# d9d-project/d9d

Measured on AMD Instinct MI355X. Metric: tokens/sec (whole node), Qwen3-MoE pretrain, higher is better.
Workload: dtype bf16; 1 GPU; model=qwen3-moe-16L-768h-128e-top8 (reference example/qwen3_moe/pretrain.json), global_batch=128, seq_len=4096, microbatch=8, parallelism=dp1, optimizer=StochasticAdamW bf16+SR, engine=raw

## Files before the change

d9d_amd/csrc/attention.hip:

```cpp
#include "common.h"
#include "mfma.h"

#include <torch/extension.h>
#include <ATen/hip/HIPContext.h>

#include <type_traits>

namespace d9d {

constexpr int kFwdQ = 128;
constexpr int kFwdKv = 64;
constexpr int kBwdQ = 64;
constexpr int kBwdKv = 128;
constexpr int kBwdThreads = 512;
constexpr float kLog2e = 1.44269504088896340736f;

template <int D>
constexpr int swz_rm_mask() {
  constexpr int mask = D == 128 ? 15 : (D == 64 ? 7 : 3);
  static_assert((D * 2) % (16 * (mask + 1)) == 0, "swizzle leaves its LDS row");
  return mask;
}

template <int D, typename Byte>
D9D_DEVICE Byte* swz_rm_at(Byte* tile, int row, int col) {
  return tile + row * (D * 2) + ((col * 2) ^ ((row & swz_rm_mask<D>()) << 4));
}

template <int ROWS, typename Byte>
D9D_DEVICE Byte* swz_t_at(Byte* tile, int d, int r) {
  static_assert((ROWS * 2) % (16 << 3) == 0, "swizzle leaves its LDS row");
  return tile + d * (ROWS * 2) + ((r * 2) ^ ((d & 7) << 4));
}

template <int D, int BLOCK = 256>
D9D_DEVICE void transpose_lds_tile(bf16_t* dst, const bf16_t* src_rm, int tid) {
  for (int idx = tid; idx < (64 / 4) * (D / 2); idx += BLOCK) {
    const int d0 = (idx / 16) * 2;
    const int rb = (idx % 16) * 4;
    bf16x4_bits c0, c1;
#pragma unroll
    for (int i = 0; i < 4; ++i) {
      const uint32_t pair = *reinterpret_cast<const uint32_t*>(
          swz_rm_at<D>(reinterpret_cast<const char*>(src_rm), rb + i, d0));
      c0.s[i] = (ushort)(pair & 0xffffu);
      c1.s[i] = (ushort)(pair >> 16);
    }
    *reinterpret_cast<uint64_t*>(
        swz_t_at<64>(reinterpret_cast<char*>(dst), d0, rb)) = c0.u;
    *reinterpret_cast<uint64_t*>(
        swz_t_at<64>(reinterpret_cast<char*>(dst), d0 + 1, rb)) = c1.u;
  }
}

template <int D>
D9D_DEVICE void load_transposed_block(
    bf16x4_bits& c0, bf16x4_bits& c1, const bf16_t* src, int64_t row_stride,
    int row_lo, int row0, int row_clamp, int idx) {
  const int d0 = (idx % (D / 2)) * 2;
  const int rb = (idx / (D / 2)) * 4;
#pragma unroll
  for (int i = 0; i < 4; ++i) {
    const int g_row = row_lo + min(row0 + rb + i, row_clamp);
    const uint32_t pair = *reinterpret_cast<const uint32_t*>(
        src + (int64_t)g_row * row_stride + d0);
    c0.s[i] = (ushort)(pair & 0xffffu);
    c1.s[i] = (ushort)(pair >> 16);
  }
}

template <int D, int ROWS>
D9D_DEVICE void store_transposed_block(
    bf16_t* dst, const bf16x4_bits& c0, const bf16x4_bits& c1, int idx) {
  const int d0 = (idx % (D / 2)) * 2;
  const int rb = (idx / (D / 2)) * 4;
  *reinterpret_cast<uint64_t*>(
      swz_t_at<ROWS>(reinterpret_cast<char*>(dst), d0, rb)) = c0.u;
  *reinterpret_cast<uint64_t*>(
      swz_t_at<ROWS>(reinterpret_cast<char*>(dst), d0 + 1, rb)) = c1.u;
}

template <int D, int ROWS, int BLOCK>
D9D_DEVICE void stage_transposed_tile(
    bf16_t* dst, const bf16_t* src, int64_t row_stride,
    int row_lo, int row0, int row_clamp, int tid) {
  for (int idx = tid; idx < (ROWS / 4) * (D / 2); idx += BLOCK) {
    bf16x4_bits c0, c1;
    load_transposed_block<D>(c0, c1, src, row_stride, row_lo, row0, row_clamp, idx);
    store_transposed_block<D, ROWS>(dst, c0, c1, idx);
  }
}


struct TileLoc {
  int b, h, tile;
  int q_lo, Sq_loc, kv_lo, Skv_loc;
  int causal_off;
  bool valid;
};

template <int TILE, bool TILE_KV>
D9D_DEVICE TileLoc locate_tile(
    const int* __restrict__ cu_q, const int* __restrict__ cu_k,
    const int* __restrict__ tile_pref, int nseq,
    int Sq, int Skv, int Hq, int q_offset) {
  TileLoc t;
  if (cu_q != nullptr) {
    t.h = blockIdx.y;
    int lo = 0, hi = nseq - 1;
    while (lo < hi) {
      const int mid = (lo + hi + 1) >> 1;
      if (tile_pref[mid] <= (int)blockIdx.x) lo = mid; else hi = mid - 1;
    }
    t.b = 0;
    t.tile = blockIdx.x - tile_pref[lo];
    t.q_lo = cu_q[lo];
    t.Sq_loc = cu_q[lo + 1] - t.q_lo;
    t.kv_lo = cu_k[lo];
    t.Skv_loc = cu_k[lo + 1] - t.kv_lo;
    t.causal_off = t.Skv_loc - t.Sq_loc + q_offset;
    t.valid = t.tile * TILE < (TILE_KV ? t.Skv_loc : t.Sq_loc);
  } else {
    const int wid = xcd_remap(blockIdx.y * gridDim.x + blockIdx.x,
                              gridDim.x * gridDim.y);
    const int bh = wid / gridDim.x;
    t.b = bh / Hq;
    t.h = bh % Hq;
    t.tile = wid % gridDim.x;
    t.q_lo = 0; t.Sq_loc = Sq; t.kv_lo = 0; t.Skv_loc = Skv;
    t.causal_off = q_offset;
    t.valid = true;
  }
  return t;
}

D9D_DEVICE bool causal_window_masked(bool masked, int q_pos, int kv_pos,
                                     int causal, int window_left) {
  if (causal) masked |= kv_pos > q_pos;
  if (window_left >= 0) masked |= kv_pos < q_pos - window_left;
  return masked;
}


template <int D>
__global__ __launch_bounds__(256, 2) void flash_fwd_kernel(
    const bf16_t* __restrict__ q,
    const bf16_t* __restrict__ k,
    const bf16_t* __restrict__ v,
    bf16_t* __restrict__ out,
    float* __restrict__ lse,
    const float* __restrict__ sinks,
    const int* __restrict__ cu_q,
    const int* __restrict__ cu_k,
    const int* __restrict__ qtile_pref,
    int nseq,
    int B, int Sq, int Skv, int Hq, int Hkv,
    float scale, int causal, int window_left, int q_offset) {
  constexpr int kNT = D / 16;
  constexpr int kKS = D / 32;

  extern __shared__ __attribute__((aligned(16))) char smem[];
  bf16_t* k_lds = reinterpret_cast<bf16_t*>(smem);
  bf16_t* vt_lds = k_lds + kFwdKv * D;
  bf16_t* p_lds = vt_lds + D * kFwdKv;

  const int lane = threadIdx.x & 63;
  const int wave = threadIdx.x >> 6;

  const TileLoc loc = locate_tile<kFwdQ, false>(
      cu_q, cu_k, qtile_pref, nseq, Sq, Skv, Hq, q_offset);
  if (!loc.valid) return;
  const int b = loc.b, h = loc.h, q_tile = loc.tile, causal_off = loc.causal_off;
  const int q_lo = loc.q_lo, Sq_loc = loc.Sq_loc, kv_lo = loc.kv_lo, Skv_loc = loc.Skv_loc;
  const int hkv = h / (Hq / Hkv);

  const int64_t q_base = ((int64_t)b * Sq * Hq + h) * D;
  const int64_t kv_base = ((int64_t)b * Skv * Hkv + hkv) * D;
  const int64_t q_row_stride = (int64_t)Hq * D;
  const int64_t kv_row_stride = (int64_t)Hkv * D;

  bf16x8 q_frag[2][kKS];
#pragma unroll
  for (int m = 0; m < 2; ++m) {
    const int q_row_local = q_tile * kFwdQ + wave * 32 + m * 16 + (lane & 15);
    const int safe_row = q_lo + min(q_row_local, Sq_loc - 1);
    const bf16_t* qp = q + q_base + (int64_t)safe_row * q_row_stride;
#pragma unroll
    for (int ks = 0; ks < kKS; ++ks) {
      q_frag[m][ks] = *reinterpret_cast<const bf16x8*>(qp + ks * 32 + (lane >> 4) * 8);
    }
  }

  const float m_init = sinks ? sinks[h] : -1e30f;
  const float l_init = (sinks && (threadIdx.x & 15) == 0) ? 1.f : 0.f;
  float m_run[2][4], l_run[2][4];
#pragma unroll
  for (int m = 0; m < 2; ++m)
#pragma unroll
    for (int r = 0; r < 4; ++r) {
      m_run[m][r] = m_init;
      l_run[m][r] = l_init;
    }
  f32x4 o_acc[2][kNT];
#pragma unroll
  for (int m = 0; m < 2; ++m)
#pragma unroll
    for (int nt = 0; nt < kNT; ++nt) o_acc[m][nt] = {0.f, 0.f, 0.f, 0.f};

  const int q_tile_last_row = min(q_tile * kFwdQ + kFwdQ - 1, Sq_loc - 1);
  int kv_end = Skv_loc;
  if (causal) kv_end = min(Skv_loc, q_tile_last_row + causal_off + 1);
  const int num_kv_tiles = (kv_end + kFwdKv - 1) / kFwdKv;
  if (num_kv_tiles <= 0) return;

  constexpr int kKIters = (kFwdKv * D) / (256 * 8);
  constexpr int kVIters = (kFwdKv / 4) * (D / 2) / 256;
  bf16x8 k_reg[kKIters];
  bf16x4_bits v_c0[kVIters], v_c1[kVIters];

  auto load_regs = [&](int kt) {
    const int kv0 = kt * kFwdKv;
#pragma unroll
    for (int it = 0; it < kKIters; ++it) {
      const int idx = (threadIdx.x + it * 256) * 8;
      const int row = idx / D;
      const int col = idx % D;
      const int g_row = kv_lo + min(kv0 + row, Skv_loc - 1);
      k_reg[it] = *reinterpret_cast<const bf16x8*>(
          k + kv_base + (int64_t)g_row * kv_row_stride + col);
    }
#pragma unroll
    for (int it = 0; it < kVIters; ++it) {
      load_transposed_block<D>(v_c0[it], v_c1[it], v + kv_base, kv_row_stride,
                               kv_lo, kv0, Skv_loc - 1, threadIdx.x + it * 256);
    }
  };

  auto store_lds = [&]() {
#pragma unroll
    for (int it = 0; it < kKIters; ++it) {
      const int idx = (threadIdx.x + it * 256) * 8;
      *reinterpret_cast<bf16x8*>(
          swz_rm_at<D>(reinterpret_cast<char*>(k_lds), idx / D, idx % D)) =
          k_reg[it];
    }
#pragma unroll
    for (int it = 0; it < kVIters; ++it) {
      store_transposed_block<D, kFwdKv>(vt_lds, v_c0[it], v_c1[it],
                                        threadIdx.x + it * 256);
    }
  };

  load_regs(0);
  store_lds();
  __syncthreads();

  for (int kt = 0; kt < num_kv_tiles; ++kt) {
    const int kv0 = kt * kFwdKv;
    if (kt + 1 < num_kv_tiles) load_regs(kt + 1);

#pragma unroll
    for (int m = 0; m < 2; ++m) {
      f32x4 s_acc[4];
#pragma unroll
      for (int nt = 0; nt < 4; ++nt) s_acc[nt] = {0.f, 0.f, 0.f, 0.f};
      __builtin_amdgcn_s_setprio(1);
#pragma unroll
      for (int nt = 0; nt < 4; ++nt) {
        const int kv_row = nt * 16 + (lane & 15);
#pragma unroll
        for (int ks = 0; ks < kKS; ++ks) {
          const int d0 = ks * 32 + (lane >> 4) * 8;
          const bf16x8 kb = *reinterpret_cast<const bf16x8*>(
              swz_rm_at<D>(reinterpret_cast<char*>(k_lds), kv_row, d0));
          s_acc[nt] = mfma16(q_frag[m][ks], kb, s_acc[nt]);
        }
      }
      __builtin_amdgcn_s_setprio(0);

      const int my_q_row = q_tile * kFwdQ + wave * 32 + m * 16;
      float p_val[4][4];
      float m_new[4];
#pragma unroll
      for (int r = 0; r < 4; ++r) m_new[r] = m_run[m][r];
      const int row_lo = my_q_row + causal_off;
      const bool any_mask =
          (kv0 + kFwdKv > kv_end) ||
          (causal && kv0 + kFwdKv - 1 > row_lo) ||
          (window_left >= 0 && kv0 < row_lo + 15 - window_left);
      if (any_mask) {
#pragma unroll
        for (int nt = 0; nt < 4; ++nt) {
          const int col = kv0 + nt * 16 + (lane & 15);
#pragma unroll
          for (int r = 0; r < 4; ++r) {
            const int row = my_q_row + (lane >> 4) * 4 + r + causal_off;
            float s = s_acc[nt][r] * scale;
            const bool masked = causal_window_masked(
                col >= kv_end, row, col, causal, window_left);
            p_val[nt][r] = masked ? -1e30f : s;
          }
        }
      } else {
#pragma unroll
        for (int nt = 0; nt < 4; ++nt)
#pragma unroll
          for (int r = 0; r < 4; ++r) p_val[nt][r] = s_acc[nt][r] * scale;
      }
#pragma unroll
      for (int r = 0; r < 4; ++r) {
        float mx = fmaxf(fmaxf(p_val[0][r], p_val[1][r]),
                         fmaxf(p_val[2][r], p_val[3][r]));
#pragma unroll
        for (int off = 1; off < 16; off <<= 1) {
          mx = fmaxf(mx, __shfl_xor(mx, off, 64));
        }
        m_new[r] = fmaxf(m_new[r], mx);
      }
      float l_add[4];
#pragma unroll
      for (int r = 0; r < 4; ++r) {
        float acc = 0.f;
#pragma unroll
        for (int nt = 0; nt < 4; ++nt) {
          const float p = __builtin_amdgcn_exp2f((p_val[nt][r] - m_new[r]) * kLog2e);
          p_val[nt][r] = p;
          acc += p;
        }
        l_add[r] = acc;
      }
      bool same = true;
#pragma unroll
      for (int r = 0; r < 4; ++r) same &= (m_new[r] == m_run[m][r]);
      if (__all(same)) {
#pragma unroll
        for (int r = 0; r < 4; ++r) l_run[m][r] += l_add[r];
      } else {
#pragma unroll
        for (int r = 0; r < 4; ++r) {
          const float alpha = __builtin_amdgcn_exp2f((m_run[m][r] - m_new[r]) * kLog2e);
          l_run[m][r] = l_run[m][r] * alpha + l_add[r];
          m_run[m][r] = m_new[r];
#pragma unroll
          for (int nt = 0; nt < kNT; ++nt) o_acc[m][nt][r] *= alpha;
        }
      }

      {
        bf16_t* pw = p_lds + (wave * 32 + m * 16) * (kFwdKv + 8);
#pragma unroll
        for (int nt = 0; nt < 4; ++nt) {
#pragma unroll
          for (int r = 0; r < 4; ++r) {
            const int row = (lane >> 4) * 4 + r;
            const int col = nt * 16 + (lane & 15);
            pw[row * (kFwdKv + 8) + col] = (bf16_t)p_val[nt][r];
          }
        }
        const bf16_t* pr = pw;
        __builtin_amdgcn_s_setprio(1);
#pragma unroll
        for (int ks2 = 0; ks2 < 2; ++ks2) {
          const int kv_off = ks2 * 32 + (lane >> 4) * 8;
          const bf16x8 pa = *reinterpret_cast<const bf16x8*>(
              pr + (lane & 15) * (kFwdKv + 8) + kv_off);
#pragma unroll
          for (int nt = 0; nt < kNT; ++nt) {
            const int d = nt * 16 + (lane & 15);
            const bf16x8 vb = *reinterpret_cast<const bf16x8*>(
                swz_t_at<kFwdKv>(reinterpret_cast<char*>(vt_lds), d, kv_off));
            o_acc[m][nt] = mfma16(pa, vb, o_acc[m][nt]);
          }
        }
        __builtin_amdgcn_s_setprio(0);
      }
    }
    __syncthreads();
    if (kt + 1 < num_kv_tiles) {
      store_lds();
      __syncthreads();
    }
  }

#pragma unroll
  for (int m = 0; m < 2; ++m)
#pragma unroll
    for (int r = 0; r < 4; ++r)
#pragma unroll
      for (int off = 1; off < 16; off <<= 1)
        l_run[m][r] += __shfl_xor(l_run[m][r], off, 64);
  {
    bf16_t* o_lds = k_lds;
#pragma unroll
    for (int half = 0; half < 2; ++half) {
      __syncthreads();
      if ((wave >> 1) == half) {
#pragma unroll
        for (int m = 0; m < 2; ++m) {
#pragma unroll
          for (int r = 0; r < 4; ++r) {
            const float inv_l = (l_run[m][r] > 0.f) ? 1.f / l_run[m][r] : 0.f;
            const int row = (wave & 1) * 32 + m * 16 + (lane >> 4) * 4 + r;
#pragma unroll
            for (int nt = 0; nt < kNT; ++nt) {
              o_lds[row * D + nt * 16 + (lane & 15)] =
                  (bf16_t)(o_acc[m][nt][r] * inv_l);
            }
          }
        }
      }
      __syncthreads();
      constexpr int elems = 64 * D;
      for (int idx = threadIdx.x * 8; idx < elems; idx += 256 * 8) {
        const int row = idx / D;
        const int col = idx % D;
        const int rg = q_tile * kFwdQ + half * 64 + row;
        if (rg < Sq_loc) {
          *reinterpret_cast<bf16x8*>(
              out + q_base + (int64_t)(q_lo + rg) * q_row_stride + col) =
              *reinterpret_cast<const bf16x8*>(o_lds + row * D + col);
        }
      }
    }
    if ((lane & 15) == 0) {
#pragma unroll
      for (int m = 0; m < 2; ++m) {
#pragma unroll
        for (int r = 0; r < 4; ++r) {
          const int rg = q_tile * kFwdQ + wave * 32 + m * 16 + (lane >> 4) * 4 + r;
          if (rg < Sq_loc) {
            lse[((int64_t)b * Hq + h) * Sq + q_lo + rg] =
                m_run[m][r] + __logf(fmaxf(l_run[m][r], 1e-30f));
          }
        }
      }
    }
  }
}

template <int D>
constexpr size_t fwd_smem_bytes() {
  return sizeof(bf16_t) * (kFwdKv * D + D * kFwdKv + kFwdQ * (kFwdKv + 8));
}


__global__ void attn_delta_kernel(
    const bf16_t* __restrict__ dout,
    const bf16_t* __restrict__ out,
    float* __restrict__ delta,
    int B, int Sq, int Hq, int D) {
  const int64_t row = blockIdx.x;
  if (row >= (int64_t)B * Sq * Hq) return;
  const int h = row % Hq;
  const int s = (row / Hq) % Sq;
  const int b = row / ((int64_t)Hq * Sq);
  const bf16_t* dp = dout + row * D;
  const bf16_t* op = out + row * D;
  float acc = 0.f;
  for (int i = threadIdx.x; i < D; i += 64) {
    acc += (float)dp[i] * (float)op[i];
  }
  acc = wave_reduce_sum(acc);
  if (threadIdx.x == 0) {
    delta[((int64_t)b * Hq + h) * Sq + s] = acc;
  }
}

constexpr int kBwdXStride = (kBwdKv / 16) * 128 + 32;

template <int D>
constexpr size_t bwd_smem_bytes() {
  return sizeof(bf16_t) * (4 * kBwdQ * D + D * kBwdKv) + 2 * (kBwdQ / 4) * kBwdXStride;
}

template <int D>
__global__ __launch_bounds__(512, 1) void flash_bwd_kernel(
    const bf16_t* __restrict__ q,
    const bf16_t* __restrict__ k,
    const bf16_t* __restrict__ v,
    const bf16_t* __restrict__ dout,
    const float* __restrict__ lse,
    const float* __restrict__ delta,
    float* __restrict__ dq,
    float* __restrict__ dk,
    float* __restrict__ dv,
    const int* __restrict__ cu_q,
    const int* __restrict__ cu_k,
    const int* __restrict__ kvtile_pref,
    int nseq,
    int B, int Sq, int Skv, int Hq, int Hkv,
    float scale, int causal, int window_left, int q_offset) {
  constexpr int kNT = D / 16;
  constexpr int kKS = D / 32;
  static_assert(kNT >= 2 && kNT % 2 == 0, "dQ splits the head dim in halves");

  extern __shared__ __attribute__((aligned(16))) char smem[];
  bf16_t* q_lds = reinterpret_cast<bf16_t*>(smem);
  bf16_t* do_lds = q_lds + kBwdQ * D;
  bf16_t* tdo_lds = do_lds + kBwdQ * D;
  bf16_t* tq_lds = tdo_lds + D * kBwdQ;
  bf16_t* kt_lds = tq_lds + D * kBwdQ;
  constexpr int kXqStride = kBwdXStride;
  char* x1_lds = reinterpret_cast<char*>(kt_lds + D * kBwdKv);
  char* x2_lds = x1_lds + (kBwdQ / 4) * kXqStride;

  const int lane = threadIdx.x & 63;
  const int wave = threadIdx.x >> 6;

  const TileLoc loc = locate_tile<kBwdKv, true>(
      cu_q, cu_k, kvtile_pref, nseq, Sq, Skv, Hq, q_offset);
  if (!loc.valid || loc.Sq_loc <= 0) return;
  const int b = loc.b, h = loc.h, kv_tile = loc.tile, causal_off = loc.causal_off;
  const int q_lo = loc.q_lo, Sq_loc = loc.Sq_loc, kv_lo = loc.kv_lo, Skv_loc = loc.Skv_loc;
  const int hkv = h / (Hq / Hkv);

  const int64_t q_base = ((int64_t)b * Sq * Hq + h) * D;
  const int64_t kv_base = ((int64_t)b * Skv * Hkv + hkv) * D;
  const int64_t q_row_stride = (int64_t)Hq * D;
  const int64_t kv_row_stride = (int64_t)Hkv * D;
  const float* lse_row = lse + ((int64_t)b * Hq + h) * Sq + q_lo;
  const float* delta_row = delta + ((int64_t)b * Hq + h) * Sq + q_lo;

  const int kv0 = kv_tile * kBwdKv;

  const int kv_row_local = lane & 15;
// ... 199 lines not shown
      }
      __builtin_amdgcn_s_setprio(0);
    }

    {
      constexpr int kNTH = kNT / 2;
      const int q_mt = wave & 3;
      const int nt0 = (wave >> 2) * kNTH;
      f32x4 dq_acc[kNTH];
#pragma unroll
      for (int nt = 0; nt < kNTH; ++nt) dq_acc[nt] = {0.f, 0.f, 0.f, 0.f};
      const int q_row = q_mt * 16 + (lane & 15);
      const size_t qbase = (size_t)(q_row >> 2) * kXqStride + (q_row & 3) * 32;
      __builtin_amdgcn_s_setprio(1);
#pragma unroll
      for (int ks2 = 0; ks2 < kBwdKv / 32; ++ks2) {
        const int kv_off = ks2 * 32 + (lane >> 4) * 8;
        const bf16x8 da = *reinterpret_cast<const bf16x8*>(
            x2_lds + qbase + (kv_off >> 4) * 128 + (kv_off & 15) * 2);
#pragma unroll
        for (int nt = 0; nt < kNTH; ++nt) {
          const int d = (nt0 + nt) * 16 + (lane & 15);
          const bf16x8 kb = *reinterpret_cast<const bf16x8*>(
              swz_t_at<kBwdKv>(reinterpret_cast<char*>(kt_lds), d, kv_off));
          dq_acc[nt] = mfma16(da, kb, dq_acc[nt]);
        }
      }
      __builtin_amdgcn_s_setprio(0);
#pragma unroll
      for (int r = 0; r < 4; ++r) {
        const int q_glob = qt + q_mt * 16 + (lane >> 4) * 4 + r;
        if (q_glob < Sq_loc) {
#pragma unroll
          for (int nt = 0; nt < kNTH; ++nt) {
            atomicAdd(dq + q_base +
                          (int64_t)(q_lo + q_glob) * q_row_stride +
                          (nt0 + nt) * 16 + (lane & 15),
                      dq_acc[nt][r]);
          }
        }
      }
    }
    if (qt + kBwdQ < Sq_loc) {
      store_qdo_lds();
    }
    __syncthreads();
  }

#pragma unroll
  for (int r = 0; r < 4; ++r) {
    const int kv_glob = kv0 + wave * 16 + (lane >> 4) * 4 + r;
    if (kv_glob < Skv_loc) {
#pragma unroll
      for (int nt = 0; nt < kNT; ++nt) {
        const int d = nt * 16 + (lane & 15);
        atomicAdd(dk + kv_base + (int64_t)(kv_lo + kv_glob) * kv_row_stride + d,
                  dk_acc[nt][r]);
        atomicAdd(dv + kv_base + (int64_t)(kv_lo + kv_glob) * kv_row_stride + d,
                  dv_acc[nt][r]);
      }
    }
  }
}

__global__ void mfma_selfcheck_kernel(
    const bf16_t* __restrict__ a,
    const bf16_t* __restrict__ b,
    float* __restrict__ c) {
  const int lane = threadIdx.x & 63;
  bf16x8 af, bf;
#pragma unroll
  for (int j = 0; j < 8; ++j) {
    af[j] = a[(lane & 15) * 32 + (lane >> 4) * 8 + j];
    bf[j] = b[((lane >> 4) * 8 + j) * 16 + (lane & 15)];
  }
  f32x4 acc = {0.f, 0.f, 0.f, 0.f};
  acc = mfma16(af, bf, acc);
#pragma unroll
  for (int r = 0; r < 4; ++r) {
    c[((lane >> 4) * 4 + r) * 16 + (lane & 15)] = acc[r];
  }
}

__global__ void cast3_f32_bf16_kernel(
    const float* __restrict__ a, const float* __restrict__ b,
    const float* __restrict__ c,
    ushort* __restrict__ oa, ushort* __restrict__ ob, ushort* __restrict__ oc,
    int64_t na, int64_t nb, int64_t nc) {
  const int64_t total = na + nb + nc;
  const int64_t stride = (int64_t)gridDim.x * blockDim.x * 8;
  for (int64_t i = ((int64_t)blockIdx.x * blockDim.x + threadIdx.x) * 8;
       i < total; i += stride) {
    const float* src;
    ushort* dst;
    int64_t off = i;
    if (off < na) {
      src = a; dst = oa;
    } else if (off < na + nb) {
      src = b; dst = ob; off -= na;
    } else {
      src = c; dst = oc; off -= na + nb;
    }
    f32x4 lo = *reinterpret_cast<const f32x4*>(src + off);
    f32x4 hi = *reinterpret_cast<const f32x4*>(src + off + 4);
    bf16x4_bits p0, p1;
#pragma unroll
    for (int j = 0; j < 4; ++j) {
      p0.s[j] = bf16_bits((bf16_t)lo[j]);
      p1.s[j] = bf16_bits((bf16_t)hi[j]);
    }
    *reinterpret_cast<uint64_t*>(dst + off) = p0.u;
    *reinterpret_cast<uint64_t*>(dst + off + 4) = p1.u;
  }
}

}


namespace {

int padded_head_dim(int d) {
  for (int cand : {32, 64, 96, 128}) {
    if (d <= cand) return cand;
  }
  TORCH_CHECK(false, "head_dim too large: ", d);
  return -1;
}

torch::Tensor maybe_pad_d(torch::Tensor t, int D_pad) {
  const int D = t.size(-1);
  if (D == D_pad) return t.contiguous();
  auto padded = torch::zeros(
      {t.size(0), t.size(1), t.size(2), (int64_t)D_pad}, t.options());
  padded.narrow(-1, 0, D).copy_(t);
  return padded;
}

struct VarlenMeta {
  torch::Tensor cu_q, cu_k, pref;
  const int *cu_q_ptr = nullptr, *cu_k_ptr = nullptr, *pref_ptr = nullptr;
  int nseq = 0, n_tiles = 0;
};

VarlenMeta prepare_varlen(const c10::optional<torch::Tensor>& cu_seqlens_q,
                          const c10::optional<torch::Tensor>& cu_seqlens_k,
                          int tile, bool tile_kv, c10::Device device) {
  VarlenMeta m;
  if (!cu_seqlens_q.has_value()) return m;
  auto cu_q_cpu = cu_seqlens_q->to(torch::kInt32).cpu().contiguous();
  auto cu_k_cpu = cu_seqlens_k->to(torch::kInt32).cpu().contiguous();
  m.nseq = cu_q_cpu.numel() - 1;
  auto pref = torch::empty({m.nseq + 1}, torch::dtype(torch::kInt32));
  const int* cu = (tile_kv ? cu_k_cpu : cu_q_cpu).data_ptr<int>();
  int* p = pref.data_ptr<int>();
  for (int i = 0; i < m.nseq; ++i) {
    p[i] = m.n_tiles;
    m.n_tiles += (cu[i + 1] - cu[i] + tile - 1) / tile;
  }
  p[m.nseq] = m.n_tiles;
  m.cu_q = cu_q_cpu.to(device, true);
  m.cu_k = cu_k_cpu.to(device, true);
  m.pref = pref.to(device, true);
  m.cu_q_ptr = m.cu_q.data_ptr<int>();
  m.cu_k_ptr = m.cu_k.data_ptr<int>();
  m.pref_ptr = m.pref.data_ptr<int>();
  return m;
// ... 107 lines not shown
  auto f32opt = q.options().dtype(torch::kFloat32);
  auto delta = torch::empty({B, Hq, Sq}, f32opt);
  auto dq32 = torch::empty({B, Sq, Hq, D_pad}, f32opt);
  auto dk32 = torch::empty({B, Skv, Hkv, D_pad}, f32opt);
  auto dv32 = torch::empty({B, Skv, Hkv, D_pad}, f32opt);

  auto stream = at::hip::getCurrentHIPStream();
  hipMemsetAsync(dq32.data_ptr(), 0, dq32.numel() * sizeof(float), stream);
  hipMemsetAsync(dk32.data_ptr(), 0, dk32.numel() * sizeof(float), stream);
  hipMemsetAsync(dv32.data_ptr(), 0, dv32.numel() * sizeof(float), stream);
  {
    const int64_t rows = (int64_t)B * Sq * Hq;
    hipLaunchKernelGGL(d9d::attn_delta_kernel, dim3(rows), dim3(64), 0, stream,
                       reinterpret_cast<const __bf16*>(dop.data_ptr()),
                       reinterpret_cast<const __bf16*>(op.data_ptr()),
                       delta.data_ptr<float>(), B, Sq, Hq, D_pad);
  }
  if (dlse.has_value()) {
    auto g = dlse->to(torch::kFloat32);
    if (varlen) g = g.unsqueeze(0);
    TORCH_CHECK(g.is_cuda() && g.sizes() == delta.sizes(),
                "flash_attn_bwd: dlse must have the layout of lse");
    delta.sub_(g);
  }

  const dim3 grid(varlen ? vl.n_tiles : (Skv + d9d::kBwdKv - 1) / d9d::kBwdKv,
                  varlen ? Hq : B * Hq);
  dispatch_head_dim(D_pad, [&](auto dp) {
    constexpr int DP = decltype(dp)::value;
    hipLaunchKernelGGL((d9d::flash_bwd_kernel<DP>), grid,
                       dim3(d9d::kBwdThreads), d9d::bwd_smem_bytes<DP>(), stream,
                       reinterpret_cast<const __bf16*>(qp.data_ptr()),
                       reinterpret_cast<const __bf16*>(kp.data_ptr()),
                       reinterpret_cast<const __bf16*>(vp.data_ptr()),
                       reinterpret_cast<const __bf16*>(dop.data_ptr()),
                       lse.data_ptr<float>(), delta.data_ptr<float>(),
                       dq32.data_ptr<float>(), dk32.data_ptr<float>(),
                       dv32.data_ptr<float>(), vl.cu_q_ptr, vl.cu_k_ptr,
                       vl.pref_ptr, vl.nseq, B, Sq, Skv, Hq, Hkv,
                       (float)softmax_scale, causal ? 1 : 0, (int)window_left,
                       (int)q_offset);
  });

  torch::Tensor dq, dk, dv;
  if (D == D_pad) {
    auto bf = q.options().dtype(torch::kBFloat16);
    dq = torch::empty(dq32.sizes(), bf);
    dk = torch::empty(dk32.sizes(), bf);
    dv = torch::empty(dv32.sizes(), bf);
    const int64_t na = dq32.numel(), nb = dk32.numel(), nc = dv32.numel();
    const int64_t groups = (na + nb + nc) / 8;
    const int blocks = (int)std::min<int64_t>((groups + 255) / 256, 16384);
    hipLaunchKernelGGL(d9d::cast3_f32_bf16_kernel, dim3(blocks), dim3(256), 0,
                       stream, dq32.data_ptr<float>(), dk32.data_ptr<float>(),
                       dv32.data_ptr<float>(),
                       reinterpret_cast<ushort*>(dq.data_ptr()),
                       reinterpret_cast<ushort*>(dk.data_ptr()),
                       reinterpret_cast<ushort*>(dv.data_ptr()),
                       na, nb, nc);
  } else {
    dq = dq32.narrow(-1, 0, D).to(torch::kBFloat16).contiguous();
    dk = dk32.narrow(-1, 0, D).to(torch::kBFloat16).contiguous();
    dv = dv32.narrow(-1, 0, D).to(torch::kBFloat16).contiguous();
  }
  if (varlen) {
    dq = dq.squeeze(0);
    dk = dk.squeeze(0);
    dv = dv.squeeze(0);
  }
  return {dq, dk, dv};
}

torch::Tensor mfma_selfcheck(torch::Tensor a, torch::Tensor b) {
  TORCH_CHECK(a.sizes() == torch::IntArrayRef({16, 32}));
  TORCH_CHECK(b.sizes() == torch::IntArrayRef({32, 16}));
  auto c = torch::empty({16, 16}, a.options().dtype(torch::kFloat32));
  auto stream = at::hip::getCurrentHIPStream();
  hipLaunchKernelGGL(d9d::mfma_selfcheck_kernel, dim3(1), dim3(64), 0, stream,
                     reinterpret_cast<const __bf16*>(a.contiguous().data_ptr()),
                     reinterpret_cast<const __bf16*>(b.contiguous().data_ptr()),
                     c.data_ptr<float>());
  return c;
}
```

d9d_amd/csrc/bindings.cpp:

```cpp
#include <torch/extension.h>

std::vector<torch::Tensor> rms_norm_fwd(torch::Tensor x, torch::Tensor w, double eps, bool zero_centered);
std::vector<torch::Tensor> rms_norm_bwd(torch::Tensor x, torch::Tensor w, torch::Tensor dy, torch::Tensor inv_rms, bool zero_centered);

torch::Tensor silu_mul_fwd(torch::Tensor a, torch::Tensor b);
torch::Tensor silu_mul_packed_fwd(torch::Tensor x);
torch::Tensor silu_mul_packed_bwd(torch::Tensor x, torch::Tensor g);
std::vector<torch::Tensor> silu_mul_bwd(torch::Tensor a, torch::Tensor b, torch::Tensor g);

void copy_fp32_to_bf16_stochastic_(torch::Tensor dst, torch::Tensor src, int64_t seed);
void add_bf16_into_f32_(torch::Tensor acc, torch::Tensor x);
void adamw_stochastic_bf16_(torch::Tensor p, torch::Tensor g, torch::Tensor m, torch::Tensor v,
                            double lr, double beta1, double beta2, double eps, double weight_decay,
                            int64_t step, int64_t seed);

std::vector<torch::Tensor> flash_attn_fwd(torch::Tensor q, torch::Tensor k, torch::Tensor v,
                                           c10::optional<torch::Tensor> sinks,
                                           c10::optional<torch::Tensor> cu_seqlens_q,
                                           c10::optional<torch::Tensor> cu_seqlens_k,
                                          bool causal, double softmax_scale, int64_t window_left,
                                          int64_t q_offset);
std::vector<torch::Tensor> flash_attn_bwd(torch::Tensor dout, torch::Tensor q, torch::Tensor k,
                                          torch::Tensor v, torch::Tensor out, torch::Tensor lse,
                                          c10::optional<torch::Tensor> cu_seqlens_q,
                                          c10::optional<torch::Tensor> cu_seqlens_k,
                                          bool causal, double softmax_scale, int64_t window_left,
                                          int64_t q_offset, c10::optional<torch::Tensor> dlse);
torch::Tensor mfma_selfcheck(torch::Tensor a, torch::Tensor b);

std::vector<torch::Tensor> router_topk_fwd(torch::Tensor logits, c10::optional<torch::Tensor> bias,
                                           int64_t K, bool renormalize);
torch::Tensor router_topk_bwd(torch::Tensor logits, torch::Tensor top_idx, torch::Tensor dtop,
                              bool renormalize);

torch::Tensor causal_conv_silu_fwd(torch::Tensor x, torch::Tensor w);
std::vector<torch::Tensor> causal_conv_silu_bwd(torch::Tensor x, torch::Tensor w,
                                                torch::Tensor dy);
std::vector<torch::Tensor> gdn_chunk_fwd(torch::Tensor q, torch::Tensor k,
                                         torch::Tensor v, torch::Tensor beta,
                                         torch::Tensor decay_log,
                                         bool return_state, bool return_aux,
                                         bool skip_out);
std::vector<torch::Tensor> gdn_chunk_bwd_scan(torch::Tensor q, torch::Tensor k,
                                              torch::Tensor dout,
                                              torch::Tensor beta,
                                              torch::Tensor decay_log);
torch::Tensor causal_conv_silu_varlen_fwd(torch::Tensor x, torch::Tensor w,
                                          torch::Tensor cu_seqlens);
std::vector<torch::Tensor> causal_conv_silu_varlen_bwd(torch::Tensor x, torch::Tensor w,
                                                       torch::Tensor dy,
                                                       torch::Tensor cu_seqlens);
std::vector<torch::Tensor> gdn_chunk_fwd_varlen(torch::Tensor q, torch::Tensor k,
                                                torch::Tensor v, torch::Tensor beta,
                                                torch::Tensor decay_log,
                                                torch::Tensor cu_seqlens,
                                                bool return_state, bool return_aux,
                                                bool skip_out);
std::vector<torch::Tensor> gdn_chunk_bwd_scan_varlen(torch::Tensor q, torch::Tensor k,
                                                     torch::Tensor dout,
                                                     torch::Tensor beta,
                                                     torch::Tensor decay_log,
                                                     torch::Tensor cu_seqlens);

torch::Tensor cce_dlogits_(torch::Tensor logits, torch::Tensor lse, torch::Tensor targets,
                           torch::Tensor dl, c10::optional<torch::Tensor> dlse,
                           int64_t vocab_start, int64_t ignore_index,
                           double filter_eps);

void adamw_stochastic_bf16_multi_(
    std::vector<torch::Tensor> params, std::vector<torch::Tensor> grads,
    std::vector<torch::Tensor> exp_avgs, std::vector<torch::Tensor> exp_avg_sqs,
    double lr, double beta1, double beta2, double eps, double weight_decay,
    std::vector<int64_t> steps, std::vector<int64_t> seeds);

torch::Tensor gmm(torch::Tensor a, torch::Tensor b, torch::Tensor batch_sizes);
torch::Tensor gmm_nt(torch::Tensor a, torch::Tensor w, torch::Tensor batch_sizes);
torch::Tensor gmm_db(torch::Tensor a, torch::Tensor g, torch::Tensor batch_sizes, int64_t num_experts);

std::vector<torch::Tensor> rope_qk(torch::Tensor q, torch::Tensor k,
                                   torch::Tensor cos_t, torch::Tensor sin_t, double sin_sign);

std::vector<torch::Tensor> cce_fwd(torch::Tensor e, torch::Tensor c, torch::Tensor targets);

torch::Tensor moe_gather_rows(torch::Tensor src, torch::Tensor idx, c10::optional<torch::Tensor> scale);
torch::Tensor moe_csr_combine(torch::Tensor expert_out, c10::optional<torch::Tensor> probs,
                              torch::Tensor inv, int64_t T, int64_t K);
torch::Tensor moe_row_dot(torch::Tensor grad_out, torch::Tensor expert_out, torch::Tensor row_to_token);

PYBIND11_MODULE(TORCH_EXTENSION_NAME, m) {
  m.def("router_topk_fwd", &router_topk_fwd, "fused MoE router fwd");
  m.def("router_topk_bwd", &router_topk_bwd, "fused MoE router bwd");
  m.def("cce_dlogits_", &cce_dlogits_, "fused CCE dlogits (in-place)");
  m.def("causal_conv_silu_fwd", &causal_conv_silu_fwd, "fused causal depthwise conv + SiLU fwd");
  m.def("causal_conv_silu_bwd", &causal_conv_silu_bwd, "fused causal depthwise conv + SiLU bwd");
  m.def("gdn_chunk_fwd", &gdn_chunk_fwd, "chunked gated delta rule forward (GDN)");
  m.def("gdn_chunk_bwd_scan", &gdn_chunk_bwd_scan,
        "chunked gated delta rule backward reverse scan (GDN)");
  m.def("causal_conv_silu_varlen_fwd", &causal_conv_silu_varlen_fwd,
        "fused causal depthwise conv + SiLU fwd, packed documents");
  m.def("causal_conv_silu_varlen_bwd", &causal_conv_silu_varlen_bwd,
        "fused causal depthwise conv + SiLU bwd, packed documents");
  m.def("gdn_chunk_fwd_varlen", &gdn_chunk_fwd_varlen,
        "chunked gated delta rule forward, packed documents (GDN)");
  m.def("gdn_chunk_bwd_scan_varlen", &gdn_chunk_bwd_scan_varlen,
        "chunked gated delta rule backward reverse scan, packed documents (GDN)");
  m.def("adamw_stochastic_bf16_multi_", &adamw_stochastic_bf16_multi_, "multi-tensor fused SR-AdamW");
  m.def("gmm", &gmm, "CDNA4 grouped GEMM (MoE experts)");
  m.def("gmm_nt", &gmm_nt, "CDNA4 grouped GEMM, weight (E,N,K)");
  m.def("gmm_db", &gmm_db, "CDNA4 grouped GEMM weight-grad");
  m.def("rope_qk", &rope_qk, "fused q/k rotary embedding");
  m.def("cce_fwd", &cce_fwd, "fused linear cross-entropy forward (lse, target logit, lse of the bf16-rounded logits)");
  m.def("moe_gather_rows", &moe_gather_rows, "MoE row gather (optional scale)");
  m.def("moe_csr_combine", &moe_csr_combine, "MoE weighted replica combine");
  m.def("moe_row_dot", &moe_row_dot, "per-row dot for prob grads");
  m.def("flash_attn_fwd", &flash_attn_fwd, "CDNA4 flash attention forward");
  m.def("flash_attn_bwd", &flash_attn_bwd, "CDNA4 flash attention backward");
  m.def("mfma_selfcheck", &mfma_selfcheck, "MFMA fragment-map self check");
  m.def("rms_norm_fwd", &rms_norm_fwd, "RMSNorm forward (bf16, CDNA4)");
  m.def("rms_norm_bwd", &rms_norm_bwd, "RMSNorm backward (bf16, CDNA4)");
  m.def("silu_mul_fwd", &silu_mul_fwd, "fused silu(a)*b forward");
  m.def("silu_mul_packed_fwd", &silu_mul_packed_fwd, "packed SwiGLU fwd");
  m.def("silu_mul_packed_bwd", &silu_mul_packed_bwd, "packed SwiGLU bwd");
  m.def("silu_mul_bwd", &silu_mul_bwd, "fused silu(a)*b backward");
  m.def("add_bf16_into_f32_", &add_bf16_into_f32_,
        "acc(fp32) += x(bf16), single pass");
  m.def("copy_fp32_to_bf16_stochastic_", &copy_fp32_to_bf16_stochastic_,
        "stochastic-rounding fp32->bf16 copy");
  m.def("adamw_stochastic_bf16_", &adamw_stochastic_bf16_,
        "fused AdamW step with SR bf16 param writes");
}
```

Before: 136,100 tokens/s.

## Keep attention P in registers via transposed S and permuted K rows

Flash attention forward now computes S transposed (K as A operand, Q as B) and permutes K rows when staging them. The softmax output is then laid out in registers exactly as the B operand of the PV MFMA, so the P round trip through LDS is gone and that LDS allocation is dropped. Row max and sum reductions become fewer cross-lane shuffles, the output is staged through swizzled LDS, and non-varlen causal Q tiles are scheduled in reverse order so the heaviest tiles start first. An MFMA chaining self-check is added to validate the fragment mapping; the risk is subtle layout or masking errors and higher register pressure.

```diff
diff --git a/d9d_amd/csrc/attention.hip b/d9d_amd/csrc/attention.hip
--- a/d9d_amd/csrc/attention.hip
+++ b/d9d_amd/csrc/attention.hip
@@ -68,6 +68,25 @@
     c1.s[i] = (ushort)(pair >> 16);
   }
 }
+
+constexpr int pv_pos(int p) {
+  return (p & ~31) | ((p & 12) << 1) | ((p & 16) >> 2) | (p & 3);
+}
+
+constexpr bool pv_pos_is_unit_permutation() {
+  bool seen[64] = {};
+  for (int p = 0; p < 64; ++p) {
+    const int kv = pv_pos(p);
+    if (kv < 0 || kv >= 64 || seen[kv]) return false;
+    seen[kv] = true;
+    if (kv != pv_pos(p & ~3) + (p & 3) || pv_pos(p & ~3) % 4 != 0) return false;
+    const int b = kv >> 5, g = (kv >> 3) & 3, j = kv & 7;
+    if (p != 32 * b + 16 * (j >> 2) + 4 * g + (j & 3)) return false;
+  }
+  return true;
+}
+static_assert(pv_pos_is_unit_permutation(),
+              "pv_pos must permute 0..63 in aligned 4-row units");
 
 template <int D, int ROWS>
 D9D_DEVICE void store_transposed_block(
@@ -126,7 +145,7 @@
     const int bh = wid / gridDim.x;
     t.b = bh / Hq;
     t.h = bh % Hq;
-    t.tile = wid % gridDim.x;
+    t.tile = TILE_KV ? wid % gridDim.x : gridDim.x - 1 - wid % gridDim.x;
     t.q_lo = 0; t.Sq_loc = Sq; t.kv_lo = 0; t.Skv_loc = Skv;
     t.causal_off = q_offset;
     t.valid = true;
@@ -162,10 +181,12 @@
   extern __shared__ __attribute__((aligned(16))) char smem[];
   bf16_t* k_lds = reinterpret_cast<bf16_t*>(smem);
   bf16_t* vt_lds = k_lds + kFwdKv * D;
-  bf16_t* p_lds = vt_lds + D * kFwdKv;
 
   const int lane = threadIdx.x & 63;
   const int wave = threadIdx.x >> 6;
+  const int lrow = lane & 15;
+  const int lgrp = lane >> 4;
+  const bool upper = lane >= 32;
 
   const TileLoc loc = locate_tile<kFwdQ, false>(
       cu_q, cu_k, qtile_pref, nseq, Sq, Skv, Hq, q_offset);
@@ -182,25 +203,24 @@
   bf16x8 q_frag[2][kKS];
 #pragma unroll
   for (int m = 0; m < 2; ++m) {
-    const int q_row_local = q_tile * kFwdQ + wave * 32 + m * 16 + (lane & 15);
+    const int q_row_local = q_tile * kFwdQ + wave * 32 + m * 16 + lrow;
     const int safe_row = q_lo + min(q_row_local, Sq_loc - 1);
     const bf16_t* qp = q + q_base + (int64_t)safe_row * q_row_stride;
 #pragma unroll
     for (int ks = 0; ks < kKS; ++ks) {
-      q_frag[m][ks] = *reinterpret_cast<const bf16x8*>(qp + ks * 32 + (lane >> 4) * 8);
+      q_frag[m][ks] = *reinterpret_cast<const bf16x8*>(qp + ks * 32 + lgrp * 8);
     }
   }
 
   const float m_init = sinks ? sinks[h] : -1e30f;
-  const float l_init = (sinks && (threadIdx.x & 15) == 0) ? 1.f : 0.f;
-  float m_run[2][4], l_run[2][4];
-#pragma unroll
-  for (int m = 0; m < 2; ++m)
-#pragma unroll
-    for (int r = 0; r < 4; ++r) {
-      m_run[m][r] = m_init;
-      l_run[m][r] = l_init;
-    }
+  const float l_init = (sinks && lgrp == 0) ? 1.f : 0.f;
+  float m_run[2], l_run[2][4];
+#pragma unroll
+  for (int m = 0; m < 2; ++m) {
+    m_run[m] = m_init;
+#pragma unroll
+    for (int r = 0; r < 4; ++r) l_run[m][r] = r == 0 ? l_init : 0.f;
+  }
   f32x4 o_acc[2][kNT];
 #pragma unroll
   for (int m = 0; m < 2; ++m)
@@ -225,7 +245,7 @@
       const int idx = (threadIdx.x + it * 256) * 8;
       const int row = idx / D;
       const int col = idx % D;
-      const int g_row = kv_lo + min(kv0 + row, Skv_loc - 1);
+      const int g_row = kv_lo + min(kv0 + pv_pos(row), Skv_loc - 1);
       k_reg[it] = *reinterpret_cast<const bf16x8*>(
           k + kv_base + (int64_t)g_row * kv_row_stride + col);
     }
@@ -259,122 +279,115 @@
     const int kv0 = kt * kFwdKv;
     if (kt + 1 < num_kv_tiles) load_regs(kt + 1);
 
+    f32x4 st[2][4];
+#pragma unroll
+    for (int m = 0; m < 2; ++m)
+#pragma unroll
+      for (int nt = 0; nt < 4; ++nt) st[m][nt] = {0.f, 0.f, 0.f, 0.f};
+    __builtin_amdgcn_s_setprio(1);
+#pragma unroll
+    for (int nt = 0; nt < 4; ++nt) {
+      const int kv_row = nt * 16 + lrow;
+#pragma unroll
+      for (int ks = 0; ks < kKS; ++ks) {
+        const int d0 = ks * 32 + lgrp * 8;
+        const bf16x8 ka = *reinterpret_cast<const bf16x8*>(
+            swz_rm_at<D>(reinterpret_cast<char*>(k_lds), kv_row, d0));
+#pragma unroll
+        for (int m = 0; m < 2; ++m) st[m][nt] = mfma16(ka, q_frag[m][ks], st[m][nt]);
+      }
+    }
+    __builtin_amdgcn_s_setprio(0);
+
+    bf16x8 pb[2][2];
 #pragma unroll
     for (int m = 0; m < 2; ++m) {
-      f32x4 s_acc[4];
-#pragma unroll
-      for (int nt = 0; nt < 4; ++nt) s_acc[nt] = {0.f, 0.f, 0.f, 0.f};
-      __builtin_amdgcn_s_setprio(1);
-#pragma unroll
-      for (int nt = 0; nt < 4; ++nt) {
-        const int kv_row = nt * 16 + (lane & 15);
-#pragma unroll
-        for (int ks = 0; ks < kKS; ++ks) {
-          const int d0 = ks * 32 + (lane >> 4) * 8;
-          const bf16x8 kb = *reinterpret_cast<const bf16x8*>(
-              swz_rm_at<D>(reinterpret_cast<char*>(k_lds), kv_row, d0));
-          s_acc[nt] = mfma16(q_frag[m][ks], kb, s_acc[nt]);
-        }
-      }
-      __builtin_amdgcn_s_setprio(0);
-
       const int my_q_row = q_tile * kFwdQ + wave * 32 + m * 16;
-      float p_val[4][4];
-      float m_new[4];
-#pragma unroll
-      for (int r = 0; r < 4; ++r) m_new[r] = m_run[m][r];
       const int row_lo = my_q_row + causal_off;
       const bool any_mask =
           (kv0 + kFwdKv > kv_end) ||
           (causal && kv0 + kFwdKv - 1 > row_lo) ||
           (window_left >= 0 && kv0 < row_lo + 15 - window_left);
       if (any_mask) {
+        const int row = row_lo + lrow;
 #pragma unroll
         for (int nt = 0; nt < 4; ++nt) {
-          const int col = kv0 + nt * 16 + (lane & 15);
 #pragma unroll
           for (int r = 0; r < 4; ++r) {
-            const int row = my_q_row + (lane >> 4) * 4 + r + causal_off;
-            float s = s_acc[nt][r] * scale;
+            const int col = kv0 + pv_pos(nt * 16 + lgrp * 4 + r);
             const bool masked = causal_window_masked(
                 col >= kv_end, row, col, causal, window_left);
-            p_val[nt][r] = masked ? -1e30f : s;
+            st[m][nt][r] = masked ? -1e30f : st[m][nt][r] * scale;
           }
         }
       } else {
 #pragma unroll
         for (int nt = 0; nt < 4; ++nt)
 #pragma unroll
-          for (int r = 0; r < 4; ++r) p_val[nt][r] = s_acc[nt][r] * scale;
-      }
+          for (int r = 0; r < 4; ++r) st[m][nt][r] = st[m][nt][r] * scale;
+      }
+      float mx = st[m][0][0];
+#pragma unroll
+      for (int nt = 0; nt < 4; ++nt)
+#pragma unroll
+        for (int r = 0; r < 4; ++r) mx = fmaxf(mx, st[m][nt][r]);
+      mx = fmaxf(mx, __shfl_xor(mx, 16, 64));
+      mx = fmaxf(mx, __shfl_xor(mx, 32, 64));
+      const float m_new = fmaxf(m_run[m], mx);
+#pragma unroll
+      for (int nt = 0; nt < 4; ++nt)
+#pragma unroll
+        for (int r = 0; r < 4; ++r)
+          st[m][nt][r] = __builtin_amdgcn_exp2f((st[m][nt][r] - m_new) * kLog2e);
+      float l_add[4];
 #pragma unroll
       for (int r = 0; r < 4; ++r) {
-        float mx = fmaxf(fmaxf(p_val[0][r], p_val[1][r]),
-                         fmaxf(p_val[2][r], p_val[3][r]));
-#pragma unroll
-        for (int off = 1; off < 16; off <<= 1) {
-          mx = fmaxf(mx, __shfl_xor(mx, off, 64));
-        }
-        m_new[r] = fmaxf(m_new[r], mx);
-      }
-      float l_add[4];
-#pragma unroll
-      for (int r = 0; r < 4; ++r) {
-        float acc = 0.f;
-#pragma unroll
-        for (int nt = 0; nt < 4; ++nt) {
-          const float p = __builtin_amdgcn_exp2f((p_val[nt][r] - m_new[r]) * kLog2e);
-          p_val[nt][r] = p;
-          acc += p;
-        }
-        l_add[r] = acc;
-      }
-      bool same = true;
-#pragma unroll
-      for (int r = 0; r < 4; ++r) same &= (m_new[r] == m_run[m][r]);
-      if (__all(same)) {
+        const float give0 = upper ? st[m][0][r] : st[m][1][r];
+        const float give1 = upper ? st[m][2][r] : st[m][3][r];
+        const float got0 = __shfl_xor(give0, 32, 64);
+        const float got1 = __shfl_xor(give1, 32, 64);
+        const float own0 = upper ? st[m][1][r] : st[m][0][r];
+        const float a2 = upper ? got1 : st[m][2][r];
+        const float a3 = upper ? st[m][3][r] : got1;
+        l_add[r] = ((own0 + got0) + a2) + a3;
+      }
+      if (__all(m_new == m_run[m])) {
 #pragma unroll
         for (int r = 0; r < 4; ++r) l_run[m][r] += l_add[r];
       } else {
-#pragma unroll
-        for (int r = 0; r < 4; ++r) {
-          const float alpha = __builtin_amdgcn_exp2f((m_run[m][r] - m_new[r]) * kLog2e);
-          l_run[m][r] = l_run[m][r] * alpha + l_add[r];
-          m_run[m][r] = m_new[r];
-#pragma unroll
-          for (int nt = 0; nt < kNT; ++nt) o_acc[m][nt][r] *= alpha;
+        const float alpha = __builtin_amdgcn_exp2f((m_run[m] - m_new) * kLog2e);
+#pragma unroll
+        for (int r = 0; r < 4; ++r) l_run[m][r] = l_run[m][r] * alpha + l_add[r];
+        m_run[m] = m_new;
+#pragma unroll
+        for (int nt = 0; nt < kNT; ++nt)
+#pragma unroll
+          for (int r = 0; r < 4; ++r) o_acc[m][nt][r] *= alpha;
+      }
+#pragma unroll
+      for (int ks2 = 0; ks2 < 2; ++ks2)
+#pragma unroll
+        for (int j = 0; j < 4; ++j) {
+          pb[m][ks2][j] = (bf16_t)st[m][2 * ks2][j];
+          pb[m][ks2][4 + j] = (bf16_t)st[m][2 * ks2 + 1][j];
         }
-      }
-
-      {
-        bf16_t* pw = p_lds + (wave * 32 + m * 16) * (kFwdKv + 8);
-#pragma unroll
-        for (int nt = 0; nt < 4; ++nt) {
-#pragma unroll
-          for (int r = 0; r < 4; ++r) {
-            const int row = (lane >> 4) * 4 + r;
-            const int col = nt * 16 + (lane & 15);
-            pw[row * (kFwdKv + 8) + col] = (bf16_t)p_val[nt][r];
-          }
-        }
-        const bf16_t* pr = pw;
-        __builtin_amdgcn_s_setprio(1);
-#pragma unroll
-        for (int ks2 = 0; ks2 < 2; ++ks2) {
-          const int kv_off = ks2 * 32 + (lane >> 4) * 8;
-          const bf16x8 pa = *reinterpret_cast<const bf16x8*>(
-              pr + (lane & 15) * (kFwdKv + 8) + kv_off);
-#pragma unroll
-          for (int nt = 0; nt < kNT; ++nt) {
-            const int d = nt * 16 + (lane & 15);
-            const bf16x8 vb = *reinterpret_cast<const bf16x8*>(
-                swz_t_at<kFwdKv>(reinterpret_cast<char*>(vt_lds), d, kv_off));
-            o_acc[m][nt] = mfma16(pa, vb, o_acc[m][nt]);
-          }
-        }
-        __builtin_amdgcn_s_setprio(0);
-      }
-    }
+    }
+
+    __builtin_amdgcn_s_setprio(1);
+#pragma unroll
+    for (int ks2 = 0; ks2 < 2; ++ks2) {
+      const int kv_off = ks2 * 32 + lgrp * 8;
+#pragma unroll
+      for (int nt = 0; nt < kNT; ++nt) {
+        const int d = nt * 16 + lrow;
+        const bf16x8 va = *reinterpret_cast<const bf16x8*>(
+            swz_t_at<kFwdKv>(reinterpret_cast<char*>(vt_lds), d, kv_off));
+#pragma unroll
+        for (int m = 0; m < 2; ++m) o_acc[m][nt] = mfma16(va, pb[m][ks2], o_acc[m][nt]);
+      }
+    }
+    __builtin_amdgcn_s_setprio(0);
+
     __syncthreads();
     if (kt + 1 < num_kv_tiles) {
       store_lds();
@@ -383,29 +396,29 @@
   }
 
 #pragma unroll
-  for (int m = 0; m < 2; ++m)
-#pragma unroll
-    for (int r = 0; r < 4; ++r)
-#pragma unroll
-      for (int off = 1; off < 16; off <<= 1)
-        l_run[m][r] += __shfl_xor(l_run[m][r], off, 64);
+  for (int m = 0; m < 2; ++m) {
+    l_run[m][0] = (l_run[m][0] + l_run[m][1]) + (l_run[m][2] + l_run[m][3]);
+    l_run[m][0] += __shfl_xor(l_run[m][0], 32, 64);
+    l_run[m][0] += __shfl_xor(l_run[m][0], 16, 64);
+  }
   {
-    bf16_t* o_lds = k_lds;
+    char* o_lds = reinterpret_cast<char*>(k_lds);
 #pragma unroll
     for (int half = 0; half < 2; ++half) {
       __syncthreads();
       if ((wave >> 1) == half) {
 #pragma unroll
         for (int m = 0; m < 2; ++m) {
-#pragma unroll
-          for (int r = 0; r < 4; ++r) {
-            const float inv_l = (l_run[m][r] > 0.f) ? 1.f / l_run[m][r] : 0.f;
-            const int row = (wave & 1) * 32 + m * 16 + (lane >> 4) * 4 + r;
-#pragma unroll
-            for (int nt = 0; nt < kNT; ++nt) {
-              o_lds[row * D + nt * 16 + (lane & 15)] =
-                  (bf16_t)(o_acc[m][nt][r] * inv_l);
-            }
+          const float inv_l = (l_run[m][0] > 0.f) ? 1.f / l_run[m][0] : 0.f;
+          const int row = (wave & 1) * 32 + m * 16 + lrow;
+#pragma unroll
+          for (int nt = 0; nt < kNT; ++nt) {
+            bf16x4_bits o4;
+#pragma unroll
+            for (int r = 0; r < 4; ++r)
+              o4.s[r] = bf16_bits((bf16_t)(o_acc[m][nt][r] * inv_l));
+            *reinterpret_cast<uint64_t*>(
+                swz_rm_at<D>(o_lds, row, nt * 16 + lgrp * 4)) = o4.u;
           }
         }
       }
@@ -418,20 +431,17 @@
         if (rg < Sq_loc) {
           *reinterpret_cast<bf16x8*>(
               out + q_base + (int64_t)(q_lo + rg) * q_row_stride + col) =
-              *reinterpret_cast<const bf16x8*>(o_lds + row * D + col);
+              *reinterpret_cast<const bf16x8*>(swz_rm_at<D>(o_lds, row, col));
         }
       }
     }
-    if ((lane & 15) == 0) {
+    if (lgrp == 0) {
 #pragma unroll
       for (int m = 0; m < 2; ++m) {
-#pragma unroll
-        for (int r = 0; r < 4; ++r) {
-          const int rg = q_tile * kFwdQ + wave * 32 + m * 16 + (lane >> 4) * 4 + r;
-          if (rg < Sq_loc) {
-            lse[((int64_t)b * Hq + h) * Sq + q_lo + rg] =
-                m_run[m][r] + __logf(fmaxf(l_run[m][r], 1e-30f));
-          }
+        const int rg = q_tile * kFwdQ + wave * 32 + m * 16 + lrow;
+        if (rg < Sq_loc) {
+          lse[((int64_t)b * Hq + h) * Sq + q_lo + rg] =
+              m_run[m] + __logf(fmaxf(l_run[m][0], 1e-30f));
         }
       }
     }
@@ -440,7 +450,7 @@
 
 template <int D>
 constexpr size_t fwd_smem_bytes() {
-  return sizeof(bf16_t) * (kFwdKv * D + D * kFwdKv + kFwdQ * (kFwdKv + 8));
+  return sizeof(bf16_t) * (kFwdKv * D + D * kFwdKv);
 }
 
 
@@ -806,6 +816,41 @@
   }
 }
 
+__global__ void mfma_chain_selfcheck_kernel(
+    const bf16_t* __restrict__ a1,
+    const bf16_t* __restrict__ b1,
+    const bf16_t* __restrict__ a2,
+    float* __restrict__ y) {
+  const int lane = threadIdx.x & 63;
+  bf16x8 bf, a2f;
+#pragma unroll
+  for (int j = 0; j < 8; ++j) {
+    bf[j] = b1[((lane >> 4) * 8 + j) * 16 + (lane & 15)];
+    a2f[j] = a2[(lane & 15) * 32 + (lane >> 4) * 8 + j];
+  }
+  f32x4 x[2];
+#pragma unroll
+  for (int t = 0; t < 2; ++t) {
+    bf16x8 af;
+#pragma unroll
+    for (int j = 0; j < 8; ++j) {
+      af[j] = a1[pv_pos(t * 16 + (lane & 15)) * 32 + (lane >> 4) * 8 + j];
+    }
+    x[t] = mfma16(af, bf, f32x4{0.f, 0.f, 0.f, 0.f});
+  }
+  bf16x8 xb;
+#pragma unroll
+  for (int j = 0; j < 4; ++j) {
+    xb[j] = (bf16_t)x[0][j];
+    xb[4 + j] = (bf16_t)x[1][j];
+  }
+  const f32x4 acc = mfma16(a2f, xb, f32x4{0.f, 0.f, 0.f, 0.f});
+#pragma unroll
+  for (int r = 0; r < 4; ++r) {
+    y[((lane >> 4) * 4 + r) * 16 + (lane & 15)] = acc[r];
+  }
+}
+
 __global__ void cast3_f32_bf16_kernel(
     const float* __restrict__ a, const float* __restrict__ b,
     const float* __restrict__ c,
@@ -1079,3 +1124,22 @@
                      c.data_ptr<float>());
   return c;
 }
+
+torch::Tensor mfma_chain_selfcheck(torch::Tensor a1, torch::Tensor b1,
+                                   torch::Tensor a2) {
+  TORCH_CHECK(a1.sizes() == torch::IntArrayRef({32, 32}));
+  TORCH_CHECK(b1.sizes() == torch::IntArrayRef({32, 16}));
+  TORCH_CHECK(a2.sizes() == torch::IntArrayRef({16, 32}));
+  for (const auto& t : {a1, b1, a2}) {
+    TORCH_CHECK(t.is_cuda() && t.scalar_type() == torch::kBFloat16);
+  }
+  auto a1c = a1.contiguous(), b1c = b1.contiguous(), a2c = a2.contiguous();
+  auto y = torch::empty({16, 16}, a1.options().dtype(torch::kFloat32));
+  auto stream = at::hip::getCurrentHIPStream();
+  hipLaunchKernelGGL(d9d::mfma_chain_selfcheck_kernel, dim3(1), dim3(64), 0,
+                     stream, reinterpret_cast<const __bf16*>(a1c.data_ptr()),
+                     reinterpret_cast<const __bf16*>(b1c.data_ptr()),
+                     reinterpret_cast<const __bf16*>(a2c.data_ptr()),
+                     y.data_ptr<float>());
+  return y;
+}
diff --git a/d9d_amd/csrc/bindings.cpp b/d9d_amd/csrc/bindings.cpp
--- a/d9d_amd/csrc/bindings.cpp
+++ b/d9d_amd/csrc/bindings.cpp
@@ -27,6 +27,7 @@
                                           bool causal, double softmax_scale, int64_t window_left,
                                           int64_t q_offset, c10::optional<torch::Tensor> dlse);
 torch::Tensor mfma_selfcheck(torch::Tensor a, torch::Tensor b);
+torch::Tensor mfma_chain_selfcheck(torch::Tensor a1, torch::Tensor b1, torch::Tensor a2);
 
 std::vector<torch::Tensor> router_topk_fwd(torch::Tensor logits, c10::optional<torch::Tensor> bias,
                                            int64_t K, bool renormalize);
@@ -116,6 +117,8 @@
   m.def("flash_attn_fwd", &flash_attn_fwd, "CDNA4 flash attention forward");
   m.def("flash_attn_bwd", &flash_attn_bwd, "CDNA4 flash attention backward");
   m.def("mfma_selfcheck", &mfma_selfcheck, "MFMA fragment-map self check");
+  m.def("mfma_chain_selfcheck", &mfma_chain_selfcheck,
+        "MFMA chained-fragment (C registers as B operand) self check");
   m.def("rms_norm_fwd", &rms_norm_fwd, "RMSNorm forward (bf16, CDNA4)");
   m.def("rms_norm_bwd", &rms_norm_bwd, "RMSNorm backward (bf16, CDNA4)");
   m.def("silu_mul_fwd", &silu_mul_fwd, "fused silu(a)*b forward");
```

After: 139,700 tokens/s, median of 6. 2.7% higher.
